# MIT-SPARK/Kimera-Semantics

Hardware: NVIDIA B200
Metric: depth_frames_per_s (higher is better)
Workload: dtype f32

## Files before the change

include/ksg.h:

```cpp
#ifndef KSG_H_
#define KSG_H_

#include <stddef.h>
#include <stdint.h>

#ifdef __cplusplus
extern "C" {
#endif

#define KSG_ABI_VERSION 1

enum {
  KSG_OK = 0,
  KSG_ERR_INVALID_ARGUMENT = 1,
  KSG_ERR_CUDA = 2,
  KSG_ERR_POOL_FULL = 3,
  KSG_ERR_SCRATCH_FULL = 4,
  KSG_ERR_INDEX_RANGE = 5,
  KSG_ERR_NO_DEVICE = 6
};

enum { KSG_INTEGRATOR_MERGED = 0, KSG_INTEGRATOR_FAST = 1 };
enum { KSG_COLOR_MODE_COLOR = 0, KSG_COLOR_MODE_SEMANTIC = 1, KSG_COLOR_MODE_SEMANTIC_PROBABILITY = 2 };
enum { KSG_ORDER_MIXED = 0, KSG_ORDER_SORTED = 1 };
// ... 143 lines not shown

int32_t ksg_reset(ksg_integrator* h);

int32_t ksg_owner_mask(int32_t voxels_per_side, int32_t shard_rank, int32_t shard_count, int64_t n,
                       const int32_t* block_index, uint8_t* mask);

int64_t ksg_unordered_map_schedule(int64_t n, int64_t* bucket_count_after_insert);

#define KSG_NUM_PHASES 7
int32_t ksg_set_profiling(ksg_integrator* h, int32_t enable);
int32_t ksg_get_profile(ksg_integrator* h, double* phase_ms , int64_t* frames,
                        int64_t* kernel_launches , int64_t* library_calls );

int64_t ksg_debug_tile_times(ksg_integrator* h, int32_t enable, int64_t capacity, int64_t* records_and_cycles);

int64_t ksg_debug_fast_timeline(ksg_integrator* h, int64_t* out80 , int64_t* sweeps, double* clock_khz);

int32_t ksg_debug_chain_sum(const float* terms, int64_t n, float s0, float* result);

const char* ksg_build_info(void);

#ifdef __cplusplus
}
#endif
#endif
```

kimera_semantics_b200/capi.py:

```python
from __future__ import annotations

import ctypes as C
import os
from typing import Dict, Optional

import numpy as np

KSG_ABI_VERSION = 1
KSG_INTEGRATOR_MERGED = 0
KSG_INTEGRATOR_FAST = 1
KSG_COLOR_MODE_COLOR = 0
KSG_COLOR_MODE_SEMANTIC = 1
KSG_COLOR_MODE_SEMANTIC_PROBABILITY = 2
KSG_ORDER_MIXED = 0
KSG_ORDER_SORTED = 1
KSG_BUNDLE_ORDER_CANONICAL = 0
KSG_BUNDLE_ORDER_LIBSTDCXX = 1

KSG_STATUS = {0: "OK", 1: "INVALID_ARGUMENT", 2: "CUDA", 3: "POOL_FULL", 4: "SCRATCH_FULL", 5: "INDEX_RANGE",
              6: "NO_DEVICE"}


class KsgConfig(C.Structure):
    _fields_ = [
# ... 413 lines not shown

    def set_profiling(self, enable: bool):
        self._check(self.lib.ksg_set_profiling(self.handle, int(enable)), "ksg_set_profiling")

    def get_profile(self) -> Dict[str, float]:
        ms = (C.c_double * 7)()
        frames, launches, libcalls = C.c_int64(), C.c_int64(), C.c_int64()
        self._check(self.lib.ksg_get_profile(self.handle, ms, C.byref(frames), C.byref(launches), C.byref(libcalls)), "ksg_get_profile")
        out = {n: float(ms[i]) for i, n in enumerate(self.PHASES)}
        out["frames"] = int(frames.value)
        out["kernel_launches"] = int(launches.value)
        out["library_calls"] = int(libcalls.value)
        return out

    def fast_timeline(self) -> Dict[str, object]:
        out = (C.c_int64 * 80)()
        sweeps, khz = C.c_int64(), C.c_double()
        n = int(self.lib.ksg_debug_fast_timeline(self.handle, out, C.byref(sweeps), C.byref(khz)))
        if n == 0:
            return {}
        t = [int(v) for v in out]
        us = lambda a, b: (t[b] - t[a]) / (khz.value / 1e3)
        ns = int(sweeps.value)
        return {"sweeps": ns, "compact_us": us(0, 1), "ray_setup_us": us(1, 2),
                "sweep_us": [us(2 + i, 3 + i) for i in range(max(0, min(ns, 48)))],
                "commit_emit_us": us(52, 53), "tile_count_us": us(53, 54), "tile_alloc_block_init_us": us(54, 55), "scatter_us": us(55, 56),
                "solve_kernel_us": us(0, 56),
                "phase0_us": {"file_shared_slot_visitors": us(0, 57) if t[57] else None, "sort_shared_slots": us(57, 58) if t[58] else None,
                              "scan_cast_counts": us(58 if t[58] else 0, 59), "compaction": us(59, 1)},
                "debug": {"max_ray_setup_us": t[64] / (khz.value / 1e3), "max_ray_setup_insert_us": t[65] / (khz.value / 1e3),
                          "max_ray_eval_us": t[67] / (khz.value / 1e3), "ray_evals": t[68], "blocks_evaluated": t[69], "blocks_materialised": t[70],
                          "ray_evals_that_changed": t[71], "max_shared_slot_visitors": t[72], "shared_slot_visitors": t[73],
                          "shared_slots": t[74], "rays": t[75],
                          "max_setup_after_loads_us": t[76] / (khz.value / 1e3), "max_setup_after_init_us": t[77] / (khz.value / 1e3),
                          "max_setup_after_loop_us": t[78] / (khz.value / 1e3), "max_eval_first_block_loads_us": t[79] / (khz.value / 1e3)}}

    def sync(self):
        self._check(self.lib.ksg_sync(self.handle), "ksg_sync")

    def reset(self):
        self._check(self.lib.ksg_reset(self.handle), "ksg_reset")

    def num_blocks(self) -> int:
        return int(self.lib.ksg_num_blocks(self.handle))

    def export(self) -> Dict[str, np.ndarray]:
        return export_arrays(self.lib, self.handle, "ksg", self.cfg.voxels_per_side, self.cfg.num_labels)

    def import_blocks(self, exp: Dict[str, np.ndarray]):
        a = {k: np.ascontiguousarray(v) for k, v in exp.items()}
# ... 78 lines not shown
```

kimera_semantics_b200/csrc/ksg_api.cu:

```cuda
#include <cuda_runtime.h>
#include <cub/cub.cuh>

#include <algorithm>
#include <cmath>
#include <cstdio>
#include <cstring>
#include <string>
#include <unordered_map>
#include <utility>
#include <vector>

#include "../../include/ksg.h"
#include "ksg_kernels.cuh"
#include "ksg_chain.cuh"
#include "ksg_hot.cuh"
#include "ksg_bundle_order.cuh"
#include "ksg_fast.cuh"
#include "ksg_fast3.cuh"
#include "ksg_voxel.cuh"
#include "ksg_merge.cuh"
#include "ksg_eval.cuh"
#include "ksg_mesh.cuh"

using namespace ksg;
// ... 99 lines not shown
  size_t cub_temp_bytes = 0;

  uint8_t* h_stage = nullptr;
  size_t h_stage_bytes = 0;
  uint8_t* d_in = nullptr;
  size_t d_in_bytes = 0;

  uint8_t* d_exp = nullptr;
  size_t d_exp_bytes = 0;
  int* d_exp_slots = nullptr;
  int exp_slots_cap = 0;

  bool fast_v2 = false;
  FastCounters* d_fc = nullptr;
  FastCounters* h_fc = nullptr;
  int *blk_cnt = nullptr, *blk_off = nullptr, *warp_cnt = nullptr, *warp_off = nullptr, *seq_of_i = nullptr;
  uint32_t* keys32 = nullptr;
  int *tile_cnt = nullptr, *tile_slot = nullptr;
  TileDesc* tile_list = nullptr;
  int solve_grid = 0, apply_fast_smem = 0;
  int solver = 3;
  int solve_threads = kSolveThreads;
  int group0 = kGroup0, group_mul = 4;
  Cand* cand16 = nullptr;
  OvfEnt* ovf = nullptr;
  RayRec* rayrec = nullptr;
  int ovf_cap = 0;
  int *mixed_list = nullptr, *m_list = nullptr, *blk_run = nullptr;
  VoxelUpdate *d_log_head = nullptr, *h_log_head = nullptr;
  float *d_log_prior = nullptr, *h_log_prior = nullptr;
// ... 79 lines not shown
  return KSG_OK;
}

template <typename Tp>
cudaError_t dmalloc(Tp** p, size_t count) { return cudaMalloc((void**)p, std::max<size_t>(count, 1) * sizeof(Tp)); }

void free_all(ksg_integrator* h) {
  cudaSetDevice(h->device);
  void* ptrs[] = {h->map.ht_keys, h->map.ht_slot, h->map.new_list, h->map.pool, h->map.slot_key, h->map.touched_stamp,
                  h->map.touched_list, h->d_luts, h->d_cnt, h->pt_pC, h->pt_pG, h->pt_label, h->pt_flags, h->pt_color, h->pt_key,
                  h->flags8, h->is_last, h->pix_list, h->point_of_seq, h->sq_keys, h->sq_keys_out, h->iota,
                  h->start_next, h->start_min, h->clear_ff, h->clear_00, h->start_table, h->cast_seq, h->ray_param, h->ray_label, h->ray_flags,
                  h->ray_color, h->nsteps, h->H, h->L, h->ray_state, h->ext_off, h->eval_sweep, h->ob.slot_stamp, h->ob.cand_pos, h->ob.bkt, h->ob.cand_val, h->ob.cand_order,
                  h->ob.cand_next, h->ob.table, h->ks_sorted, h->seq_sorted, h->bstart, h->bundle_f, h->hist,
                  h->tmp, h->tmp4, h->b_key, h->b_base, h->bord_hash, h->bord_scratch, h->d_scan_tot, h->bundle_f2, h->d_hot_segs, h->d_hot_counts, h->d_hot_chunk_seg, h->d_hot_guess, h->d_hot_sums,
                  h->d_hot_tables, h->d_hot_prior, h->d_hot_same, h->tile_debug, h->d_gridbar, h->d_fc, h->blk_cnt, h->blk_off, h->warp_cnt, h->warp_off, h->seq_of_i, h->keys32,
                  h->tile_cnt, h->tile_slot, h->tile_list, h->cand16, h->ovf, h->rayrec, h->mixed_list, h->m_list, h->blk_run, h->stamp64, h->d_log_head, h->d_log_prior, h->vq.long_items, h->vq.counters, h->rec_a, h->rec_b, h->tile_begin, h->cub_temp, h->d_in, h->d_exp, h->d_exp_slots};
  for (void* p : ptrs) if (p) cudaFree(p);
  if (h->h_cnt_base) cudaFreeHost(h->h_cnt_base);
  if (h->h_log_head) cudaFreeHost(h->h_log_head);
  if (h->h_log_prior) cudaFreeHost(h->h_log_prior);
  if (h->h_fc_base) cudaFreeHost(h->h_fc_base);
  for (int i = 0; i < 2; ++i) {
    if (h->ev_frame_s[i]) cudaEventDestroy(h->ev_frame_s[i]);
    if (h->ev_copy[i]) cudaEventDestroy(h->ev_copy[i]);
    if (h->ev_free[i]) cudaEventDestroy(h->ev_free[i]);
    if (h->d_in2[i]) cudaFree(h->d_in2[i]);
    if (h->h_stage2[i]) cudaFreeHost(h->h_stage2[i]);
  }
  if (h->copy_stream) cudaStreamDestroy(h->copy_stream);
  if (h->ev_fork) cudaEventDestroy(h->ev_fork);
// ... 203 lines not shown
      h->set_offset = 0;
      KSG_CUDA(cudaMemsetAsync(h->start_table, 0xFF, sizeof(uint32_t) * kSetSize, s));
      KSG_CUDA(cudaMemsetAsync(h->ob.table, 0xFF, sizeof(uint32_t) * kSetSize, s));
    }
  }
  FastFrame f{};
  f.cfg = h->dc; f.T = T; f.in = fin; f.in.pix_list = nullptr; f.in.point_of_seq = nullptr;
  f.luts = h->d_luts; f.cnt = h->d_cnt; f.fc = h->d_fc; f.map = h->map; f.ob = h->ob;
  f.sb = StartBuf{h->start_head, h->start_next, h->start_min, h->start_max, h->start_val, h->start_mixed, h->start_table};
  f.set_offset = h->set_offset;
  f.capacity = cap;
  f.n_count_blocks = (cap + kCountBlock - 1) / kCountBlock;
  f.vec_ok = in.d_depth ? (((uintptr_t)in.d_depth % 16 == 0 && (uintptr_t)in.d_label_img % 4 == 0) ? 1 : 0) : 0;
  f.frame_stamp = h->frame_stamp;
  f.profile = h->profiling ? 1 : 0;
  f.seq_of_i = sorted ? h->seq_of_i : nullptr;
  f.block_cnt = h->blk_cnt; f.block_off = h->blk_off; f.warp_cnt = h->warp_cnt; f.warp_off = h->warp_off;
  f.pt_pG = h->pt_pG; f.pt_label = h->pt_label; f.pt_flags = h->pt_flags; f.pt_color = h->pt_color; f.pt_key = h->pt_key;
  f.cast_flag = h->flags8;
  f.cast_seq = h->cast_seq; f.ray_param = h->ray_param; f.ray_label = h->ray_label; f.ray_flags = h->ray_flags; f.ray_color = h->ray_color;
  f.nsteps = h->nsteps; f.H = h->H; f.L = h->L; f.ray_state = h->ray_state; f.ext_off = h->ext_off; f.eval_sweep = h->eval_sweep;
  f.rec = h->rec_a; f.rec_cap = h->rec_cap; f.keys = h->keys32;
  f.tile_cnt = h->tile_cnt; f.tile_slot = h->tile_slot; f.tile_list = h->tile_list; f.tile_cap = h->tile_cap;
  f.o3.cand = h->cand16; f.o3.ext_base = h->ob.ext_base; f.o3.cand_cap = h->ob.cand_cap; f.o3.slot_cnt = h->ob.slot_cnt; f.o3.bkt = h->ob.bkt;
  f.o3.head = h->ob.head; f.o3.ovf = h->ovf; f.o3.ovf_cap = h->ovf_cap; f.o3.stamp_max = h->stamp64; f.o3.stamp_min = h->stamp64 + kSetSize; f.o3.table = h->ob.table;
  f.rayrec = h->rayrec; f.blk_run = h->blk_run;
  f.log_head = h->d_log_head; f.log_prior = h->d_log_prior; f.log_cap = h->log_cap;
  f.group0 = h->group0; f.group_mul = h->group_mul;
  f.s_base = h->start_head; f.s_hmin = h->start_val; f.s_hmax = (uint32_t*)(h->clear_00 + (size_t)kSetSize * 5);
  f.s_visits = (int*)(h->clear_00 + (size_t)kSetSize * 9); f.mixed_list = h->mixed_list; f.m_list = h->m_list;
  const bool s3 = h->solver == 3;

  if (h->profiling) {
    cudaEventRecord(h->ev[0], s);
    KSG_CUDA(cudaMemsetAsync(h->d_fc->dbg, 0, sizeof(h->d_fc->dbg), s));
  }
  KSG_CUDA(cudaMemsetAsync(h->clear_ff, 0xFF, (size_t)kSetSize * 16, s));
  KSG_CUDA(cudaMemsetAsync(h->clear_00, 0x00, (size_t)kSetSize * (s3 ? 13 : 5), s));
  KSG_CUDA(cudaMemsetAsync(h->start_min, 0x7F, sizeof(int) * kSetSize, s));
  const int B = 256;
  ++h->n_launches;
  if (in.d_depth) k_fast_count<<<f.n_count_blocks, 256, 0, s>>>(f);
  else k_fast_reset<<<1, 1, 0, s>>>(f);
  if (sorted) {
    h->n_launches += 3;
    if (in.d_depth) k_fast_sqnorm<<<f.n_count_blocks, 256, 0, s>>>(f, h->sq_keys);
    else k_fast_sqnorm_points<<<grid_for(cap, B), B, 0, s>>>(f, h->sq_keys);
    k_fast_pad_keys<<<grid_for(cap, B), B, 0, s>>>(h->d_cnt, cap, h->sq_keys);
    size_t tb = h->cub_temp_bytes;
    ++h->n_libcalls;
// ... 1583 lines not shown
    const uint64_t key = pack_key(bi);
    for (int z = 0; z < vps; ++z)
      for (int y = 0; y < vps; ++y)
        for (int x = 0; x < vps; ++x) {
          const int tile = (x / T) + tps * ((y / T) + tps * (z / T));
          mask[b * V + (size_t)x + (size_t)vps * ((size_t)y + (size_t)vps * z)] = tile_owner(key, tile, count) == shard_rank ? 1 : 0;
        }
  }
  return KSG_OK;
}

int32_t ksg_set_profiling(ksg_integrator* h, int32_t enable) {
  if (!h) return KSG_ERR_INVALID_ARGUMENT;
  cudaSetDevice(h->device);
  if (enable && !h->ev[0]) for (auto& e : h->ev) cudaEventCreate(&e);
  h->profiling = enable != 0;
  for (double& m : h->phase_ms) m = 0.0;
  h->prof_frames = 0; h->n_launches = 0; h->n_libcalls = 0;
  return KSG_OK;
}
int32_t ksg_get_profile(ksg_integrator* h, double* phase_ms, int64_t* frames, int64_t* kernel_launches, int64_t* library_calls) {
  if (!h) return KSG_ERR_INVALID_ARGUMENT;
  if (phase_ms) for (int p = 0; p < KSG_NUM_PHASES; ++p) phase_ms[p] = h->phase_ms[p];
  if (frames) *frames = h->prof_frames;
  if (kernel_launches) *kernel_launches = h->n_launches;
  if (library_calls) *library_calls = h->n_libcalls;
  return KSG_OK;
}

namespace {
// ... 28 lines not shown
    if (cudaMalloc((void**)&h->tile_debug, sizeof(long long) * 2 * (size_t)h->tile_cap) != cudaSuccess) { h->tile_debug = nullptr; return 0; }
  }
  const int64_t n = std::min<int64_t>(h->h_cnt->n_tiles, h->tile_cap);
  if (h->tile_debug && records_and_cycles && capacity >= n && n > 0)
    cudaMemcpy(records_and_cycles, h->tile_debug, sizeof(long long) * 2 * n, cudaMemcpyDeviceToHost);
  if (!enable && h->tile_debug) { cudaFree(h->tile_debug); h->tile_debug = nullptr; }
  return n;
}

int64_t ksg_debug_fast_timeline(ksg_integrator* h, int64_t* out64, int64_t* sweeps, double* clock_khz) {
  if (!h || !out64 || !h->h_fc) return 0;
  cudaSetDevice(h->device);
  if (h->n_pend > 0) finish_frame(h, nullptr);
  for (int i = 0; i < kTimelineSlots; ++i) out64[i] = (int64_t)h->h_fc->timeline[i];
  for (int i = 0; i < 16; ++i) out64[kTimelineSlots + i] = (int64_t)h->h_fc->dbg[i];
  if (sweeps) *sweeps = h->h_fc->sweeps_last;
  if (clock_khz) *clock_khz = h->clock_khz;
  return kTimelineSlots + 16;
}

int32_t ksg_clear_map(ksg_integrator* h) {
  if (!h) return KSG_ERR_INVALID_ARGUMENT;
  auto fail = [&](int c, const char* m) { return h->fail(c, m); };
  KSG_CUDA(cudaSetDevice(h->device));
  KSG_CUDA(cudaDeviceSynchronize());
  { const int rcp = finish_frame(h, nullptr); if (rcp) return rcp; }
  cudaStream_t s = h->own_stream;
  KSG_CUDA(cudaMemsetAsync(h->map.ht_keys, 0xFF, sizeof(uint64_t) * h->ht_cap, s));
  KSG_CUDA(cudaMemsetAsync(h->map.ht_slot, 0xFF, sizeof(int) * h->ht_cap, s));
  KSG_CUDA(cudaMemsetAsync(h->map.touched_stamp, 0, sizeof(int) * h->ht_cap, s));
  if (h->tile_cnt) KSG_CUDA(cudaMemsetAsync(h->tile_cnt, 0, sizeof(int) * (size_t)h->ht_cap * h->dc.tiles_per_block, s));
  KSG_CUDA(cudaMemsetAsync(&h->d_cnt->pool_count, 0, sizeof(int), s));
  KSG_CUDA(cudaMemsetAsync(&h->d_cnt->n_blocks_touched, 0, sizeof(int), s));
// ... 17 lines not shown
```

kimera_semantics_b200/csrc/ksg_fast.cuh:

```cuda
#pragma once
#include "ksg_kernels.cuh"

namespace ksg {

static constexpr int kCountBlock = 1024;
static constexpr int kEvalBlock = 512;
static constexpr int kSolveThreads = 1024;
static constexpr int kFastKeyCap = 4096;
static constexpr int kFastPref = 1024;
static constexpr int kTimelineSlots = 64;

struct FastCounters {
  unsigned int ticket_count, ticket_eval;
  unsigned int gridbar;
  int sweep_base;
  int sweeps_last;
  int tile_cursor;
  int n_tile_list;
  int pool_base;
  unsigned long long rec_cursor;
  int ovf_count;
  int n_mixed;
  int m_cursor;
  int log_count;
  long long timeline[kTimelineSlots];
// ... 25 lines not shown
  DevCfg cfg;
  Xform T;
  FrameIn in;
  const Luts* luts;
  Counters* cnt;
  FastCounters* fc;
  MapRef map;
  ObsBuf ob;
  StartBuf sb;
  uint64_t set_offset;
  int capacity;
  int n_count_blocks;
  int vec_ok;
  int frame_stamp;
  int profile;
  const int* seq_of_i;
  int* block_cnt; int* block_off;
  int* warp_cnt; int* warp_off;
  float4* pt_pG; uint8_t* pt_label; uint8_t* pt_flags; uint32_t* pt_color; uint64_t* pt_key; uint8_t* cast_flag;
  int* cast_seq; float4* ray_param; uint8_t* ray_label; uint8_t* ray_flags; uint32_t* ray_color;
  int* nsteps; int* H; int* L; RayState* ray_state; long long* ext_off; int* eval_sweep;
  uint64_t* rec; long long rec_cap;
  uint32_t* keys;
  int* tile_cnt;
  int* tile_slot;
  TileDesc* tile_list; long long tile_cap;
  Obs3 o3;
  RayRec* rayrec;
  int* blk_run;
  int group0, group_mul;
// ... 282 lines not shown
          f.mixed_list[atomicAdd(&f.fc->n_mixed, 1)] = (int)slot;
        }
      }
    }
  }
  if (seq < f.capacity) f.cast_flag[seq] = cast;
  const unsigned m = __ballot_sync(0xffffffffu, cast != 0);
  if (lane == 0) __stcg(&f.warp_cnt[seq >> 5], __popc(m));
  if (blockIdx.x == 0 && threadIdx.x == 0) f.fc->gridbar = 0;
}

__device__ __forceinline__ void warp_sort_i32(int* a, int n, int lane) {
  int n2 = 1;
  while (n2 < n) n2 <<= 1;
  const int half = n2 >> 1;
  for (int k = 2; k <= n2; k <<= 1) {
    const int hk = k >> 1;
    for (int t = lane; t < half; t += 32) {
      const int blk = t / hk, o = t - blk * hk;
      const int i = blk * k + o, p = blk * k + (k - 1 - o);
      if (p < n) { const int x = a[i], y = a[p]; if (x > y) { a[i] = y; a[p] = x; } }
    }
    __syncwarp();
    for (int j = k >> 2; j > 0; j >>= 1) {
      for (int t = lane; t < half; t += 32) {
        const int i = (t / j) * 2 * j + (t % j), p = i + j;
        if (p < n) { const int x = a[i], y = a[p]; if (x > y) { a[i] = y; a[p] = x; } }
      }
      __syncwarp();
    }
  }
}

__device__ __forceinline__ void solve_barrier(unsigned int* bar, unsigned int& epoch) {
  __syncthreads();
  if (threadIdx.x == 0) {
    __threadfence();
    const unsigned int target = (++epoch) * gridDim.x;
    atomicAdd(bar, 1u);
    while (((volatile unsigned int*)bar)[0] < target) {}
    __threadfence();
  }
  __syncthreads();
}
__device__ __forceinline__ void dbg_max(const FastFrame& f, int k, long long v) { if (f.profile) atomicMax((unsigned long long*)&f.fc->dbg[k], (unsigned long long)v); }
__device__ __forceinline__ void dbg_add(const FastFrame& f, int k, long long v) { if (f.profile) atomicAdd((unsigned long long*)&f.fc->dbg[k], (unsigned long long)v); }
__device__ __forceinline__ void timeline_mark(const FastFrame& f, int slot) {
  if (f.profile && blockIdx.x == 0 && threadIdx.x == 0 && slot < kTimelineSlots) f.fc->timeline[slot] = clock64();
}

__device__ __forceinline__ void fast_ray_setup(const FastFrame& f, int r, int n_cast) {
  const DevCfg& cfg = f.cfg;
  int h = 0;
  if (r < n_cast) {
    const int seq = f.cast_seq[r];
    const float4 p = f.pt_pG[seq];
    const uint8_t fl = f.pt_flags[seq];
    f.ray_param[r] = p;
    f.ray_label[r] = f.pt_label[seq];
    f.ray_flags[r] = fl;
    f.ray_color[r] = f.pt_color[seq];
// ... 487 lines not shown
```

kimera_semantics_b200/csrc/ksg_fast3.cuh:

```cuda
#pragma once
#include "ksg_fast.cuh"

namespace ksg {

struct __align__(16) Cand { uint64_t vkey; int pos; int tog; };
struct __align__(16) OvfEnt { uint64_t order_perf; uint32_t hi; int next; };
struct __align__(16) RayRec { int H, L, nsteps, eval_sweep; };
static constexpr int kBkt3 = 32;
static constexpr int kOvfPending = -2;
static constexpr int kSortPerWarp = 1024;

__device__ __forceinline__ Cand ld_cand(const Cand* p) {
  const int4 v = __ldcg((const int4*)p);
  Cand c; c.vkey = ((uint64_t)(uint32_t)v.y << 32) | (uint32_t)v.x; c.pos = v.z; c.tog = v.w;
  return c;
}
__device__ __forceinline__ void st_cand(Cand* p, uint64_t vkey, int pos, int tog) {
  __stcg((int4*)p, make_int4((int)(uint32_t)vkey, (int)(uint32_t)(vkey >> 32), pos, tog));
}
__device__ __forceinline__ void st_cand_state(Cand* p, int pos, int tog) { __stcg((int2*)p + 1, make_int2(pos, tog)); }
__device__ __forceinline__ uint64_t cand_value(uint64_t vkey, uint64_t offset) { return (uint64_t)index_hash(unpack_key(vkey)) + offset; }
__device__ __forceinline__ uint64_t make_entry(bool on, uint64_t order, uint64_t v) { return (on ? kEntPerf : 0ull) | (order << 13) | (v >> kSetBits); }
__device__ __forceinline__ long long cand_index3(const Obs3& o, const long long* ext_off, int r, int s) {
  if (s < kH0) return (long long)r * kH0 + s;
// ... 3 lines not shown

static constexpr uint32_t kSweepCap = 0x7FFFFFFFu;
__device__ __forceinline__ void stamp_toggle(const Obs3& o, uint32_t slot, int sweep, int r) {
  atomicMax((unsigned long long*)&o.stamp_max[slot], ((unsigned long long)(uint32_t)sweep << 32) | (uint32_t)r);
  atomicMin((unsigned long long*)&o.stamp_min[slot], ((unsigned long long)(kSweepCap - (uint32_t)sweep) << 32) | (uint32_t)r);
}
__device__ __forceinline__ bool stamp_dirty(const Obs3& o, uint32_t slot, int last, int r) {
  const unsigned long long a = __ldcg((const unsigned long long*)&o.stamp_max[slot]);
  const unsigned long long b = __ldcg((const unsigned long long*)&o.stamp_min[slot]);
  const int sk = (int)(a >> 32);
  if (sk > last) return true;
  if (sk < last) return false;
  return !((uint32_t)(b >> 32) == kSweepCap - (uint32_t)sk && (uint32_t)a == (uint32_t)r && (uint32_t)b == (uint32_t)r);
}

__device__ __forceinline__ int cand_insert_raw(int* slot_cnt, uint64_t* bkt, int* head, OvfEnt* ovf, int ovf_cap, int* ovf_count, Counters* cnt,
                                            uint32_t slot, uint64_t entry) {
  const int idx = atomicAdd(&slot_cnt[slot], 1);
  if (idx < kBkt3) { const int pos = (int)slot * kBkt3 + idx; __stcg(&bkt[pos], entry); return pos; }
  const int id = atomicAdd(ovf_count, 1);
  if (id >= ovf_cap) { set_err(cnt, 4); return -2; }
  OvfEnt* e = &ovf[id];
  __stcg(&e->next, kOvfPending);
  __stcg(&e->order_perf, (entry & kEntPerf) | ((entry >> 13) & ((1ull << kEntOrderBits) - 1)));
  __stcg(&e->hi, (uint32_t)(entry & 0x1FFFull));
  const int old = atomicExch(&head[slot], id);
  __stcg(&e->next, old);
  return -3 - id;
}
__device__ __forceinline__ int cand_insert3(const FastFrame& f, uint32_t slot, uint64_t entry) {
  return cand_insert_raw(f.o3.slot_cnt, f.o3.bkt, f.o3.head, f.o3.ovf, f.o3.ovf_cap, &f.fc->ovf_count, f.cnt, slot, entry);
}

__device__ __forceinline__ int latest_performed_before_raw(const uint64_t* bkt, const int* slot_cnt, const int* head, const OvfEnt* ovf, int ovf_cap,
                                                        uint32_t slot, uint64_t my_order) {
  const ulonglong2* b = (const ulonglong2*)(bkt + (size_t)slot * kBkt3);
  const int total = __ldcg(&slot_cnt[slot]);
  ulonglong2 v[4];
#pragma unroll
  for (int q = 0; q < 4; ++q) v[q] = __ldcg(b + q);
  const int n = total < kBkt3 ? total : kBkt3;
  long long best = -1;
  int best_hi = -1;
#pragma unroll
  for (int q = 0; q < 4; ++q) scan_entries(v[q], 2 * q, n, my_order, best, best_hi);
#pragma unroll 1
// ... 7 lines not shown
    int guard = total - kBkt3 + 8;
#pragma unroll 1
    for (int id = __ldcg(&head[slot]); id >= 0 && id < ovf_cap && guard-- > 0; id = __ldcg(&ovf[id].next)) {
      const uint64_t op = __ldcg(&ovf[id].order_perf);
      const uint64_t eo = op & ~kEntPerf;
      if ((op & kEntPerf) && eo < my_order && (long long)eo > best) { best = (long long)eo; best_hi = (int)__ldcg(&ovf[id].hi); }
    }
  }
  return best_hi;
}
__device__ __forceinline__ int latest_performed_before3(const Obs3& o, uint32_t slot, uint64_t my_order) {
  return latest_performed_before_raw(o.bkt, o.slot_cnt, o.head, o.ovf, o.ovf_cap, slot, my_order);
}
__device__ __forceinline__ bool later_performed_exists_raw(const uint64_t* bkt, const int* slot_cnt, const int* head, const OvfEnt* ovf, int ovf_cap,
                                                        uint32_t slot, uint64_t my_order) {
  const int total = __ldcg(&slot_cnt[slot]);
  const int n = total < kBkt3 ? total : kBkt3;
  const uint64_t* b = bkt + (size_t)slot * kBkt3;
  bool later = false;
#pragma unroll 1
  for (int j = 0; j < n; ++j) {
    const uint64_t e = __ldcg(&b[j]);
    if ((e & kEntPerf) && ((e >> 13) & ((1ull << kEntOrderBits) - 1)) > my_order) later = true;
  }
  if (total > kBkt3) {
    int guard = total - kBkt3 + 8;
#pragma unroll 1
    for (int id = __ldcg(&head[slot]); id >= 0 && id < ovf_cap && !later && guard-- > 0; id = __ldcg(&ovf[id].next)) {
      const uint64_t op = __ldcg(&ovf[id].order_perf);
      if ((op & kEntPerf) && (op & ~kEntPerf) > my_order) later = true;
    }
  }
  return later;
}
__device__ __forceinline__ bool later_performed_exists3(const Obs3& o, uint32_t slot, uint64_t my_order) {
  return later_performed_exists_raw(o.bkt, o.slot_cnt, o.head, o.ovf, o.ovf_cap, slot, my_order);
}

// ... 121 lines not shown
  for (int r = r_lo + (threadIdx.x >> 5) * gridDim.x + blockIdx.x; r < r_hi; r += warps_total) {
    const int4 rr = __ldcg((const int4*)&f.rayrec[r]);
    int h = rr.x;
    const int old = rr.y, n = rr.z, last = rr.w;
    int fd = 0x7fffffff;
    if (last == 0) fd = 0;
    else {
      const int upto = (old < h - 1) ? old : h - 1;
      for (int s = lane; s <= upto; s += 32) {
        const Cand c = ld_cand(&o.cand[cand_index3(o, f.ext_off, r, s)]);
        const uint32_t slot = (uint32_t)cand_value(c.vkey, f.set_offset) & kSetMask;
        if (stamp_dirty(o, slot, last, r)) { fd = s; break; }
      }
      for (int d = 16; d > 0; d >>= 1) { const int t = __shfl_xor_sync(0xffffffffu, fd, d); fd = t < fd ? t : fd; }
    }
    if (fd == 0x7fffffff) continue;
    const long long t_eval = f.profile ? clock64() : 0;
    int n_blocks_eval = 0, n_blocks_mat = 0;
    int s0, blen;
    block_of_step(fd, s0, blen);
    long long base_ci = cand_index3(o, f.ext_off, r, s0);
    int run = (s0 == 0) ? 0 : __ldcg(&f.blk_run[base_ci >> 4]);
    int U = -1;
    while (s0 < n && U < 0) {
      const int cend = (s0 + blen < n) ? s0 + blen : n;
      ++n_blocks_eval;
      if (s0 >= h) {
        ++n_blocks_mat;
        int ok = 1;
        if (lane == 0 && s0 >= kH0 && (s0 & (s0 - 1)) == 0) {
          const int k = 31 - __clz(s0 >> 4);
// ... 39 lines not shown
      bool coll[2];
#pragma unroll
      for (int q = 0; q < 2; ++q) {
        const int s = s0 + q * 32 + lane;
        c[q].vkey = 0; c[q].pos = -2; c[q].tog = 0; v[q] = 0; coll[q] = false;
        if (s < cend) { c[q] = ld_cand(&o.cand[base_ci + q * 32 + lane]); v[q] = cand_value(c[q].vkey, f.set_offset); }
      }
#pragma unroll
      for (int q = 0; q < 2; ++q) {
        const int s = s0 + q * 32 + lane;
        if (s < cend) {
          const uint32_t slot = (uint32_t)v[q] & kSetMask;
          const uint32_t stale = o.table[slot];
          const int hi = latest_performed_before3(o, slot, ((uint64_t)r << kOrderStepBits) | (uint64_t)s);
          coll[q] = (hi >= 0) ? ((uint32_t)hi == (uint32_t)(v[q] >> kSetBits)) : (stale == (uint32_t)(v[q] >> kSetBits));
        }
      }
      const unsigned bits0 = __ballot_sync(0xffffffffu, coll[0]), bits1 = __ballot_sync(0xffffffffu, coll[1]);
      if (f.profile && lane == 0 && n_blocks_eval == 1) dbg_max(f, 15, clock64() - t_eval);
      int brk = -1;
      for (int jj = 0; s0 + jj < cend; ++jj) {
        const unsigned bit = (jj < 32) ? ((bits0 >> jj) & 1u) : ((bits1 >> (jj - 32)) & 1u);
        if (bit) ++run; else run = 0;
        if (run > cfg.maxc) { brk = s0 + jj; break; }
      }
      const int perf_end = (brk >= 0) ? brk : cend;
#pragma unroll
      for (int q = 0; q < 2; ++q) {
        const int s = s0 + q * 32 + lane;
        if (s < perf_end && s >= old)
// ... 4 lines not shown
      s0 = cend;
      if (s0 < n) { int nb; block_of_step(s0, s0, nb); blen = nb; if (s0 < h) base_ci = cand_index3(o, f.ext_off, r, s0); }
    }
    if (U < 0) U = n;
    if (U < old) {
      for (int s = U + lane; s < old; s += 32) {
        const long long ci = cand_index3(o, f.ext_off, r, s);
        Cand c = ld_cand(&o.cand[ci]);
        const uint64_t v = cand_value(c.vkey, f.set_offset);
        set_performed3(f, c, ci, (uint32_t)v & kSetMask, ((uint64_t)r << kOrderStepBits) | (uint64_t)s, v, false, sweep, r);
      }
    }
    if (lane == 0) {
      if (U != old) { f.rayrec[r].L = U; cnt->changed[sweep & 3] = 1; }
      f.rayrec[r].eval_sweep = sweep;
      if (f.profile) { dbg_max(f, 3, clock64() - t_eval); dbg_add(f, 4, 1); dbg_add(f, 5, n_blocks_eval); dbg_add(f, 6, n_blocks_mat); if (U != old) dbg_add(f, 7, 1); }
    }
  }
}

template <int PASS>
__device__ __forceinline__ void fast3_walk_performed(const FastFrame& f, int n_cast, int n_tiles) {
  constexpr int G = 8;
  const Obs3& o = f.o3;
  const DevCfg& cfg = f.cfg;
  const int groups_total = (gridDim.x * blockDim.x) / G;
  const int gl = threadIdx.x % G;
  const int gt = ((((threadIdx.x >> 5) * gridDim.x + blockIdx.x) << 5) | (threadIdx.x & 31));
  for (int r = gt / G; r < n_cast; r += groups_total) {
    const int U = __ldcg(&f.rayrec[r].L);
    for (int s = gl; s < U; s += G) {
// ... 21 lines not shown
        if (idx >= 0 && idx < n_tiles && at >= 0) f.keys[__ldcg(&f.tile_list[idx].off) + at] = (uint32_t)rec;
      }
    }
  }
}

__global__ void __launch_bounds__(kSolveThreads, 1) k_fast_solve3(FastFrame f, int max_sweeps) {
  unsigned int epoch = 0;
  unsigned int* bar = &f.fc->gridbar;
  const int lane = threadIdx.x & 31;
  const int gtid = (((threadIdx.x >> 5) * gridDim.x + blockIdx.x) << 5) | lane;
  const int gthreads = gridDim.x * blockDim.x;
  Counters* cnt = f.cnt;
  const int n_points = cnt->n_points;
  int tl = 0;
  timeline_mark(f, tl++);
  extern __shared__ int s_sort[];
  const int n_mixed = ((volatile int*)&f.fc->n_mixed)[0];
  if (n_mixed > 0) {
    for (int seq = gtid; seq < n_points; seq += gthreads) {
      const uint64_t v = f.pt_key[seq];
      if (v == ~0ull) continue;
      const uint32_t slot = (uint32_t)v & kSetMask;
      if (f.s_hmin[slot] != f.s_hmax[slot]) f.m_list[f.s_base[slot] + f.sb.next[seq]] = seq;
    }
    solve_barrier(bar, epoch);
    timeline_mark(f, 57);
    const int warps_total = gthreads >> 5;
    int* scratch = s_sort + (threadIdx.x >> 5) * kSortPerWarp;
    for (int mi = (threadIdx.x >> 5) * gridDim.x + blockIdx.x; mi < n_mixed; mi += warps_total) {
      const int slot = f.mixed_list[mi];
      const int n = __ldcg(&f.s_visits[slot]);
      int* seg = f.m_list + __ldcg(&f.s_base[slot]);
      int* a = seg;
      if (n <= kSortPerWarp) { for (int i = lane; i < n; i += 32) scratch[i] = __ldcg(&seg[i]); a = scratch; }
      __syncwarp();
      warp_sort_i32(a, n, lane);
      for (int i = 1 + lane; i < n; i += 32) {
        const int pa = a[i - 1], pb = a[i];
        if (f.pt_key[pa] != f.pt_key[pb]) { f.cast_flag[pb] = 1; atomicAdd(&f.warp_cnt[pb >> 5], 1); }
      }
      __syncwarp();
      if (f.profile && lane == 0) { dbg_max(f, 8, n); dbg_add(f, 9, n); }
    }
    solve_barrier(bar, epoch);
    timeline_mark(f, 58);
  }
  if (blockIdx.x == 0) {
    const int n_warps32 = (f.capacity + 31) >> 5;
    const int total = block_scan_array(f.warp_cnt, f.warp_off, n_warps32);
    if (threadIdx.x == 0) cnt->n_cast = total;
  }
  solve_barrier(bar, epoch);
  timeline_mark(f, 59);
  const int n_cast = ((volatile int*)&cnt->n_cast)[0];
  for (int base = (gtid & ~31); base < n_points; base += gthreads) {
    const int seq = base + lane;
    const bool c = seq < n_points && __ldcg(&f.cast_flag[seq]) != 0;
    const unsigned m = __ballot_sync(0xffffffffu, c);
    if (c) f.cast_seq[__ldcg(&f.warp_off[seq >> 5]) + __popc(m & ((1u << lane) - 1u))] = seq;
  }
  const int sweep_base0 = ((volatile int*)&f.fc->sweep_base)[0];
  const bool wrap = false;
  solve_barrier(bar, epoch);
  timeline_mark(f, tl++);
  for (int r0 = (gtid & ~31); r0 < n_cast; r0 += gthreads) fast3_ray_setup(f, r0 + lane, n_cast);
  solve_barrier(bar, epoch);
  timeline_mark(f, tl++);
  int sweep = (wrap ? 0 : sweep_base0);
  sweep = (sweep + 4) & ~3;
  const int first_sweep = sweep + 1;
  bool failed = false;
  int g_lo = 0, g_size = f.group0 > 0 ? f.group0 : kGroup0;
  while (g_lo < n_cast && !failed) {
    const int g_hi = (g_lo + g_size < n_cast) ? g_lo + g_size : n_cast;
    bool converged = false;
    for (int it = 0; it < max_sweeps; ++it) {
      ++sweep;
      fast3_sweep(f, sweep, g_lo, g_hi, (WarpDdaScratch*)(s_sort + (threadIdx.x >> 5) * kSortPerWarp));
      solve_barrier(bar, epoch);
      if (tl < kTimelineSlots - 12) timeline_mark(f, tl++);
      const int changed = ((volatile int*)cnt->changed)[sweep & 3];
      const int err = ((volatile int*)&cnt->err)[0];
      if (err) { failed = true; break; }
      if (!changed) { converged = true; break; }
    }
    if (!converged) failed = true;
    g_lo = g_hi;
    g_size = (g_size < (1 << 28)) ? g_size * (f.group_mul > 1 ? f.group_mul : 4) : g_size;
  }
  if (gtid == 0) {
    cnt->last_sweep = sweep;
    f.fc->sweep_base = sweep;
    f.fc->sweeps_last = sweep - first_sweep + 1;
    if (failed && !((volatile int*)&cnt->err)[0]) set_err(cnt, 2 );
    if (f.profile) f.fc->timeline[kTimelineSlots - 1] = tl;
  }
  tl = kTimelineSlots - 12;
  timeline_mark(f, tl++);
  if (!failed) fast3_walk_performed<1>(f, n_cast, 0);
  solve_barrier(bar, epoch);
  timeline_mark(f, tl++);
  timeline_mark(f, tl++);
  const bool ok = ((volatile int*)&cnt->err)[0] == 0 && !failed;
  const int n_new_all = ((volatile int*)&cnt->n_new_blocks)[0];
  const int n_new = n_new_all < f.map.new_cap ? n_new_all : f.map.new_cap;
  const int pool_base = ((volatile int*)&cnt->pool_count)[0];
  const int n_tiles = (int)min((long long)((volatile int*)&f.fc->n_tile_list)[0], f.tile_cap);
  for (int base = (gtid & ~31); base < n_tiles; base += gthreads) {
    const int idx = base + lane;
    int n = 0;
    uint32_t tk = 0;
    if (idx < n_tiles) { tk = f.tile_list[idx].tk; n = __ldcg(&f.tile_cnt[tk]); }
    const long long off = (long long)warp_alloc(&f.fc->rec_cursor, (unsigned long long)n);
    if (idx < n_tiles) {
      const int pos = (int)(tk / (uint32_t)f.cfg.tiles_per_block);
      const int old = atomicExch(&f.map.touched_stamp[pos], f.frame_stamp);
      if (old != f.frame_stamp) f.map.touched_list[atomicAdd(&cnt->n_blocks_touched, 1)] = pos;
      const bool owned = f.cfg.shard_count <= 1 ||
                         tile_owner(f.map.ht_keys[pos], (int)(tk % (uint32_t)f.cfg.tiles_per_block), f.cfg.shard_count) == f.cfg.shard_rank;
      if (off + n > f.rec_cap) { set_err(cnt, 4); n = 0; }
      f.tile_list[idx].n = owned ? n : -n;
      f.tile_list[idx].off = off;
    }
  }
  if (ok) fast_block_init(f, n_new, pool_base);
  solve_barrier(bar, epoch);
  timeline_mark(f, tl++);
  const bool ok2 = ((volatile int*)&cnt->err)[0] == 0 && !failed;
  if (!failed) fast3_walk_performed<2>(f, n_cast, ok2 ? n_tiles : 0);
  if (gtid == 0) {
    int add = n_new;
    if (pool_base + add > f.map.max_blocks) add = f.map.max_blocks - pool_base;
    if (ok) cnt->pool_count = pool_base + (add > 0 ? add : 0);
    cnt->n_tiles = ok2 ? n_tiles : 0;
    cnt->n_records = ((volatile unsigned long long*)&f.fc->rec_cursor)[0];
    f.fc->tile_cursor = 0;
    f.fc->n_tile_list = 0;
    f.fc->rec_cursor = 0;
    f.fc->ovf_count = 0;
    if (f.profile) { f.fc->dbg[10] = n_mixed; f.fc->dbg[11] = n_cast; }
    f.fc->n_mixed = 0;
    f.fc->m_cursor = 0;
    f.fc->log_count = 0;
  }
  timeline_mark(f, tl++);
}

}
```

Measured before the change: 2175.

## Add shared-memory profiling counters and vectorize slot scans and sort indexing

Profiling counters now accumulate in shared memory and are flushed once per block before each grid barrier. New per-sweep and overflow statistics are exposed through an extended timeline buffer. Separately, the bitonic warp sort replaces divisions with shifts, later_performed_exists_raw reads bucket entries as 128-bit vector loads in groups of four, and the cast-flag key comparison loop is unrolled four ways. The non-profiling changes target integer divide cost and load latency in hot loops, at the price of the bucket scan always loading eight entries even when fewer are valid.

```diff
diff --git a/include/ksg.h b/include/ksg.h
--- a/include/ksg.h
+++ b/include/ksg.h
@@ -181,7 +181,7 @@
 
 int64_t ksg_debug_tile_times(ksg_integrator* h, int32_t enable, int64_t capacity, int64_t* records_and_cycles);
 
-int64_t ksg_debug_fast_timeline(ksg_integrator* h, int64_t* out80 , int64_t* sweeps, double* clock_khz);
+int64_t ksg_debug_fast_timeline(ksg_integrator* h, int64_t* out112 , int64_t* sweeps, double* clock_khz);
 
 int32_t ksg_debug_chain_sum(const float* terms, int64_t n, float s0, float* result);
 
diff --git a/kimera_semantics_b200/capi.py b/kimera_semantics_b200/capi.py
--- a/kimera_semantics_b200/capi.py
+++ b/kimera_semantics_b200/capi.py
@@ -451,7 +451,7 @@
         return out
 
     def fast_timeline(self) -> Dict[str, object]:
-        out = (C.c_int64 * 80)()
+        out = (C.c_int64 * 112)()
         sweeps, khz = C.c_int64(), C.c_double()
         n = int(self.lib.ksg_debug_fast_timeline(self.handle, out, C.byref(sweeps), C.byref(khz)))
         if n == 0:
@@ -470,7 +470,10 @@
                           "ray_evals_that_changed": t[71], "max_shared_slot_visitors": t[72], "shared_slot_visitors": t[73],
                           "shared_slots": t[74], "rays": t[75],
                           "max_setup_after_loads_us": t[76] / (khz.value / 1e3), "max_setup_after_init_us": t[77] / (khz.value / 1e3),
-                          "max_setup_after_loop_us": t[78] / (khz.value / 1e3), "max_eval_first_block_loads_us": t[79] / (khz.value / 1e3)}}
+                          "max_setup_after_loop_us": t[78] / (khz.value / 1e3), "max_eval_first_block_loads_us": t[79] / (khz.value / 1e3),
+                          "overflow_entries": t[80], "max_slot_count": t[81], "max_overflow_chain_walked": t[82],
+                          "sweep_clean_rays": [t[84 + 2 * i] for i in range(max(0, min(ns, 14)))],
+                          "sweep_ray_evals": [t[85 + 2 * i] for i in range(max(0, min(ns, 14)))]}}
 
     def sync(self):
         self._check(self.lib.ksg_sync(self.handle), "ksg_sync")
diff --git a/kimera_semantics_b200/csrc/ksg_api.cu b/kimera_semantics_b200/csrc/ksg_api.cu
--- a/kimera_semantics_b200/csrc/ksg_api.cu
+++ b/kimera_semantics_b200/csrc/ksg_api.cu
@@ -137,6 +137,7 @@
   bool fast_v2 = false;
   FastCounters* d_fc = nullptr;
   FastCounters* h_fc = nullptr;
+  long long* d_prof = nullptr;
   int *blk_cnt = nullptr, *blk_off = nullptr, *warp_cnt = nullptr, *warp_off = nullptr, *seq_of_i = nullptr;
   uint32_t* keys32 = nullptr;
   int *tile_cnt = nullptr, *tile_slot = nullptr;
@@ -246,7 +247,7 @@
                   h->ray_color, h->nsteps, h->H, h->L, h->ray_state, h->ext_off, h->eval_sweep, h->ob.slot_stamp, h->ob.cand_pos, h->ob.bkt, h->ob.cand_val, h->ob.cand_order,
                   h->ob.cand_next, h->ob.table, h->ks_sorted, h->seq_sorted, h->bstart, h->bundle_f, h->hist,
                   h->tmp, h->tmp4, h->b_key, h->b_base, h->bord_hash, h->bord_scratch, h->d_scan_tot, h->bundle_f2, h->d_hot_segs, h->d_hot_counts, h->d_hot_chunk_seg, h->d_hot_guess, h->d_hot_sums,
-                  h->d_hot_tables, h->d_hot_prior, h->d_hot_same, h->tile_debug, h->d_gridbar, h->d_fc, h->blk_cnt, h->blk_off, h->warp_cnt, h->warp_off, h->seq_of_i, h->keys32,
+                  h->d_hot_tables, h->d_hot_prior, h->d_hot_same, h->tile_debug, h->d_gridbar, h->d_fc, h->d_prof, h->blk_cnt, h->blk_off, h->warp_cnt, h->warp_off, h->seq_of_i, h->keys32,
                   h->tile_cnt, h->tile_slot, h->tile_list, h->cand16, h->ovf, h->rayrec, h->mixed_list, h->m_list, h->blk_run, h->stamp64, h->d_log_head, h->d_log_prior, h->vq.long_items, h->vq.counters, h->rec_a, h->rec_b, h->tile_begin, h->cub_temp, h->d_in, h->d_exp, h->d_exp_slots};
   for (void* p : ptrs) if (p) cudaFree(p);
   if (h->h_cnt_base) cudaFreeHost(h->h_cnt_base);
@@ -480,6 +481,7 @@
   f.vec_ok = in.d_depth ? (((uintptr_t)in.d_depth % 16 == 0 && (uintptr_t)in.d_label_img % 4 == 0) ? 1 : 0) : 0;
   f.frame_stamp = h->frame_stamp;
   f.profile = h->profiling ? 1 : 0;
+  f.prof = h->d_prof;
   f.seq_of_i = sorted ? h->seq_of_i : nullptr;
   f.block_cnt = h->blk_cnt; f.block_off = h->blk_off; f.warp_cnt = h->warp_cnt; f.warp_off = h->warp_off;
   f.pt_pG = h->pt_pG; f.pt_label = h->pt_label; f.pt_flags = h->pt_flags; f.pt_color = h->pt_color; f.pt_key = h->pt_key;
@@ -500,6 +502,7 @@
   if (h->profiling) {
     cudaEventRecord(h->ev[0], s);
     KSG_CUDA(cudaMemsetAsync(h->d_fc->dbg, 0, sizeof(h->d_fc->dbg), s));
+    KSG_CUDA(cudaMemsetAsync(h->d_prof, 0, sizeof(long long) * kProfSlots, s));
   }
   KSG_CUDA(cudaMemsetAsync(h->clear_ff, 0xFF, (size_t)kSetSize * 16, s));
   KSG_CUDA(cudaMemsetAsync(h->clear_00, 0x00, (size_t)kSetSize * (s3 ? 13 : 5), s));
@@ -2113,6 +2116,10 @@
   if (!h) return KSG_ERR_INVALID_ARGUMENT;
   cudaSetDevice(h->device);
   if (enable && !h->ev[0]) for (auto& e : h->ev) cudaEventCreate(&e);
+  if (enable && h->d_fc && !h->d_prof) {
+    if (cudaMalloc(&h->d_prof, sizeof(long long) * kProfSlots) != cudaSuccess) { h->d_prof = nullptr; return KSG_ERR_CUDA; }
+    cudaMemset(h->d_prof, 0, sizeof(long long) * kProfSlots);
+  }
   h->profiling = enable != 0;
   for (double& m : h->phase_ms) m = 0.0;
   h->prof_frames = 0; h->n_launches = 0; h->n_libcalls = 0;
@@ -2171,9 +2178,12 @@
   if (h->n_pend > 0) finish_frame(h, nullptr);
   for (int i = 0; i < kTimelineSlots; ++i) out64[i] = (int64_t)h->h_fc->timeline[i];
   for (int i = 0; i < 16; ++i) out64[kTimelineSlots + i] = (int64_t)h->h_fc->dbg[i];
+  long long prof[kProfSlots] = {};
+  if (h->d_prof) cudaMemcpy(prof, h->d_prof, sizeof(prof), cudaMemcpyDeviceToHost);
+  for (int i = 0; i < kProfSlots; ++i) out64[kTimelineSlots + 16 + i] = (int64_t)prof[i];
   if (sweeps) *sweeps = h->h_fc->sweeps_last;
   if (clock_khz) *clock_khz = h->clock_khz;
-  return kTimelineSlots + 16;
+  return kTimelineSlots + 16 + kProfSlots;
 }
 
 int32_t ksg_clear_map(ksg_integrator* h) {
diff --git a/kimera_semantics_b200/csrc/ksg_fast.cuh b/kimera_semantics_b200/csrc/ksg_fast.cuh
--- a/kimera_semantics_b200/csrc/ksg_fast.cuh
+++ b/kimera_semantics_b200/csrc/ksg_fast.cuh
@@ -9,6 +9,8 @@
 static constexpr int kFastKeyCap = 4096;
 static constexpr int kFastPref = 1024;
 static constexpr int kTimelineSlots = 64;
+static constexpr int kProfSlots = 32;
+static constexpr int kProfSweeps = (kProfSlots - 4) / 2;
 
 struct FastCounters {
   unsigned int ticket_count, ticket_eval;
@@ -64,6 +66,7 @@
   int vec_ok;
   int frame_stamp;
   int profile;
+  long long* prof;
   const int* seq_of_i;
   int* block_cnt; int* block_off;
   int* warp_cnt; int* warp_off;
@@ -376,17 +379,18 @@
   int n2 = 1;
   while (n2 < n) n2 <<= 1;
   const int half = n2 >> 1;
-  for (int k = 2; k <= n2; k <<= 1) {
-    const int hk = k >> 1;
+  for (int lk = 1; (1 << lk) <= n2; ++lk) {
+    const int k = 1 << lk, lhk = lk - 1;
     for (int t = lane; t < half; t += 32) {
-      const int blk = t / hk, o = t - blk * hk;
+      const int blk = t >> lhk, o = t & ((1 << lhk) - 1);
       const int i = blk * k + o, p = blk * k + (k - 1 - o);
       if (p < n) { const int x = a[i], y = a[p]; if (x > y) { a[i] = y; a[p] = x; } }
     }
     __syncwarp();
-    for (int j = k >> 2; j > 0; j >>= 1) {
+    for (int lj = lk - 2; lj >= 0; --lj) {
+      const int j = 1 << lj;
       for (int t = lane; t < half; t += 32) {
-        const int i = (t / j) * 2 * j + (t % j), p = i + j;
+        const int i = ((t >> lj) << (lj + 1)) + (t & (j - 1)), p = i + j;
         if (p < n) { const int x = a[i], y = a[p]; if (x > y) { a[i] = y; a[p] = x; } }
       }
       __syncwarp();
@@ -405,8 +409,31 @@
   }
   __syncthreads();
 }
-__device__ __forceinline__ void dbg_max(const FastFrame& f, int k, long long v) { if (f.profile) atomicMax((unsigned long long*)&f.fc->dbg[k], (unsigned long long)v); }
-__device__ __forceinline__ void dbg_add(const FastFrame& f, int k, long long v) { if (f.profile) atomicAdd((unsigned long long*)&f.fc->dbg[k], (unsigned long long)v); }
+static constexpr int kDbgShared = 20;
+static constexpr unsigned kDbgAddMask = (1u << 4) | (1u << 5) | (1u << 6) | (1u << 7) | (1u << 9);
+__shared__ unsigned long long s_dbg[kDbgShared];
+__device__ __forceinline__ void dbg_max(const FastFrame& f, int k, long long v) { if (f.profile) atomicMax(&s_dbg[k], (unsigned long long)v); }
+__device__ __forceinline__ void dbg_add(const FastFrame& f, int k, long long v) { if (f.profile) atomicAdd(&s_dbg[k], (unsigned long long)v); }
+__device__ __forceinline__ void prof_init(const FastFrame& f) {
+  if (!f.profile) return;
+  if (threadIdx.x < kDbgShared) s_dbg[threadIdx.x] = 0;
+  __syncthreads();
+}
+__device__ __forceinline__ void prof_flush(const FastFrame& f, int sweep_idx) {
+  if (!f.profile) return;
+  __syncthreads();
+  const int k = threadIdx.x;
+  if (k < kDbgShared) {
+    const unsigned long long v = s_dbg[k];
+    if (v) {
+      if (k < 16) {
+        if ((kDbgAddMask >> k) & 1u) atomicAdd((unsigned long long*)&f.fc->dbg[k], v); else atomicMax((unsigned long long*)&f.fc->dbg[k], v);
+      } else if (k < 18) atomicMax((unsigned long long*)&f.prof[k - 15], v);
+      else if (sweep_idx >= 0 && sweep_idx < kProfSweeps) atomicAdd((unsigned long long*)&f.prof[4 + 2 * sweep_idx + (k - 18)], v);
+      s_dbg[k] = 0;
+    }
+  }
+}
 __device__ __forceinline__ void timeline_mark(const FastFrame& f, int slot) {
   if (f.profile && blockIdx.x == 0 && threadIdx.x == 0 && slot < kTimelineSlots) f.fc->timeline[slot] = clock64();
 }
diff --git a/kimera_semantics_b200/csrc/ksg_fast3.cuh b/kimera_semantics_b200/csrc/ksg_fast3.cuh
--- a/kimera_semantics_b200/csrc/ksg_fast3.cuh
+++ b/kimera_semantics_b200/csrc/ksg_fast3.cuh
@@ -41,22 +41,20 @@
   return !((uint32_t)(b >> 32) == kSweepCap - (uint32_t)sk && (uint32_t)a == (uint32_t)r && (uint32_t)b == (uint32_t)r);
 }
 
-__device__ __forceinline__ int cand_insert_raw(int* slot_cnt, uint64_t* bkt, int* head, OvfEnt* ovf, int ovf_cap, int* ovf_count, Counters* cnt,
-                                            uint32_t slot, uint64_t entry) {
-  const int idx = atomicAdd(&slot_cnt[slot], 1);
-  if (idx < kBkt3) { const int pos = (int)slot * kBkt3 + idx; __stcg(&bkt[pos], entry); return pos; }
-  const int id = atomicAdd(ovf_count, 1);
-  if (id >= ovf_cap) { set_err(cnt, 4); return -2; }
-  OvfEnt* e = &ovf[id];
+__device__ __forceinline__ int cand_insert3(const FastFrame& f, uint32_t slot, uint64_t entry) {
+  const Obs3& o = f.o3;
+  const int idx = atomicAdd(&o.slot_cnt[slot], 1);
+  if (f.profile) dbg_max(f, 16, idx + 1);
+  if (idx < kBkt3) { const int pos = (int)slot * kBkt3 + idx; __stcg(&o.bkt[pos], entry); return pos; }
+  const int id = atomicAdd(&f.fc->ovf_count, 1);
+  if (id >= o.ovf_cap) { set_err(f.cnt, 4); return -2; }
+  OvfEnt* e = &o.ovf[id];
   __stcg(&e->next, kOvfPending);
   __stcg(&e->order_perf, (entry & kEntPerf) | ((entry >> 13) & ((1ull << kEntOrderBits) - 1)));
   __stcg(&e->hi, (uint32_t)(entry & 0x1FFFull));
-  const int old = atomicExch(&head[slot], id);
+  const int old = atomicExch(&o.head[slot], id);
   __stcg(&e->next, old);
   return -3 - id;
-}
-__device__ __forceinline__ int cand_insert3(const FastFrame& f, uint32_t slot, uint64_t entry) {
-  return cand_insert_raw(f.o3.slot_cnt, f.o3.bkt, f.o3.head, f.o3.ovf, f.o3.ovf_cap, &f.fc->ovf_count, f.cnt, slot, entry);
 }
 
 __device__ __forceinline__ int latest_performed_before_raw(const uint64_t* bkt, const int* slot_cnt, const int* head, const OvfEnt* ovf, int ovf_cap,
@@ -94,14 +92,26 @@
 }
 __device__ __forceinline__ bool later_performed_exists_raw(const uint64_t* bkt, const int* slot_cnt, const int* head, const OvfEnt* ovf, int ovf_cap,
                                                         uint32_t slot, uint64_t my_order) {
+  const ulonglong2* b = (const ulonglong2*)(bkt + (size_t)slot * kBkt3);
   const int total = __ldcg(&slot_cnt[slot]);
+  ulonglong2 v[4];
+#pragma unroll
+  for (int q = 0; q < 4; ++q) v[q] = __ldcg(b + q);
   const int n = total < kBkt3 ? total : kBkt3;
-  const uint64_t* b = bkt + (size_t)slot * kBkt3;
   bool later = false;
 #pragma unroll 1
-  for (int j = 0; j < n; ++j) {
-    const uint64_t e = __ldcg(&b[j]);
-    if ((e & kEntPerf) && ((e >> 13) & ((1ull << kEntOrderBits) - 1)) > my_order) later = true;
+  for (int q0 = 0;;) {
+#pragma unroll
+    for (int q = 0; q < 4; ++q) {
+      const uint64_t e2[2] = {v[q].x, v[q].y};
+#pragma unroll
+      for (int k = 0; k < 2; ++k)
+        if (2 * (q0 + q) + k < n && (e2[k] & kEntPerf) && ((e2[k] >> 13) & ((1ull << kEntOrderBits) - 1)) > my_order) later = true;
+    }
+    q0 += 4;
+    if (2 * q0 >= n) break;
+#pragma unroll
+    for (int q = 0; q < 4; ++q) v[q] = __ldcg(b + q0 + q);
   }
   if (total > kBkt3) {
     int guard = total - kBkt3 + 8;
@@ -253,7 +263,7 @@
       }
       for (int d = 16; d > 0; d >>= 1) { const int t = __shfl_xor_sync(0xffffffffu, fd, d); fd = t < fd ? t : fd; }
     }
-    if (fd == 0x7fffffff) continue;
+    if (fd == 0x7fffffff) { if (f.profile && lane == 0) dbg_add(f, 18, 1); continue; }
     const long long t_eval = f.profile ? clock64() : 0;
     int n_blocks_eval = 0, n_blocks_mat = 0;
     int s0, blen;
@@ -323,6 +333,7 @@
           const uint32_t stale = o.table[slot];
           const int hi = latest_performed_before3(o, slot, ((uint64_t)r << kOrderStepBits) | (uint64_t)s);
           coll[q] = (hi >= 0) ? ((uint32_t)hi == (uint32_t)(v[q] >> kSetBits)) : (stale == (uint32_t)(v[q] >> kSetBits));
+          if (f.profile) { const int tot = __ldcg(&o.slot_cnt[slot]); if (tot > kBkt3) dbg_max(f, 17, tot - kBkt3); }
         }
       }
       const unsigned bits0 = __ballot_sync(0xffffffffu, coll[0]), bits1 = __ballot_sync(0xffffffffu, coll[1]);
@@ -357,7 +368,7 @@
     if (lane == 0) {
       if (U != old) { f.rayrec[r].L = U; cnt->changed[sweep & 3] = 1; }
       f.rayrec[r].eval_sweep = sweep;
-      if (f.profile) { dbg_max(f, 3, clock64() - t_eval); dbg_add(f, 4, 1); dbg_add(f, 5, n_blocks_eval); dbg_add(f, 6, n_blocks_mat); if (U != old) dbg_add(f, 7, 1); }
+      if (f.profile) { dbg_max(f, 3, clock64() - t_eval); dbg_add(f, 4, 1); dbg_add(f, 5, n_blocks_eval); dbg_add(f, 6, n_blocks_mat); if (U != old) dbg_add(f, 7, 1); dbg_add(f, 19, 1); }
     }
   }
 }
@@ -409,6 +420,7 @@
   Counters* cnt = f.cnt;
   const int n_points = cnt->n_points;
   int tl = 0;
+  prof_init(f);
   timeline_mark(f, tl++);
   extern __shared__ int s_sort[];
   const int n_mixed = ((volatile int*)&f.fc->n_mixed)[0];
@@ -419,6 +431,7 @@
       const uint32_t slot = (uint32_t)v & kSetMask;
       if (f.s_hmin[slot] != f.s_hmax[slot]) f.m_list[f.s_base[slot] + f.sb.next[seq]] = seq;
     }
+    prof_flush(f, -1);
     solve_barrier(bar, epoch);
     timeline_mark(f, 57);
     const int warps_total = gthreads >> 5;
@@ -428,16 +441,30 @@
       const int n = __ldcg(&f.s_visits[slot]);
       int* seg = f.m_list + __ldcg(&f.s_base[slot]);
       int* a = seg;
-      if (n <= kSortPerWarp) { for (int i = lane; i < n; i += 32) scratch[i] = __ldcg(&seg[i]); a = scratch; }
+      if (n <= kSortPerWarp) {
+#pragma unroll 4
+        for (int i = lane; i < n; i += 32) scratch[i] = __ldcg(&seg[i]);
+        a = scratch;
+      }
       __syncwarp();
       warp_sort_i32(a, n, lane);
-      for (int i = 1 + lane; i < n; i += 32) {
-        const int pa = a[i - 1], pb = a[i];
-        if (f.pt_key[pa] != f.pt_key[pb]) { f.cast_flag[pb] = 1; atomicAdd(&f.warp_cnt[pb >> 5], 1); }
+      for (int i0 = 1 + lane; i0 < n; i0 += 4 * 32) {
+        int pb[4];
+        uint64_t ka[4], kb[4];
+#pragma unroll
+        for (int u = 0; u < 4; ++u) {
+          const int i = i0 + 32 * u;
+          pb[u] = -1; ka[u] = kb[u] = 0;
+          if (i < n) { pb[u] = a[i]; ka[u] = f.pt_key[a[i - 1]]; kb[u] = f.pt_key[pb[u]]; }
+        }
+#pragma unroll
+        for (int u = 0; u < 4; ++u)
+          if (pb[u] >= 0 && ka[u] != kb[u]) { f.cast_flag[pb[u]] = 1; atomicAdd(&f.warp_cnt[pb[u] >> 5], 1); }
       }
       __syncwarp();
       if (f.profile && lane == 0) { dbg_max(f, 8, n); dbg_add(f, 9, n); }
     }
+    prof_flush(f, -1);
     solve_barrier(bar, epoch);
     timeline_mark(f, 58);
   }
@@ -446,6 +473,7 @@
     const int total = block_scan_array(f.warp_cnt, f.warp_off, n_warps32);
     if (threadIdx.x == 0) cnt->n_cast = total;
   }
+  prof_flush(f, -1);
   solve_barrier(bar, epoch);
   timeline_mark(f, 59);
   const int n_cast = ((volatile int*)&cnt->n_cast)[0];
@@ -457,9 +485,11 @@
   }
   const int sweep_base0 = ((volatile int*)&f.fc->sweep_base)[0];
   const bool wrap = false;
+  prof_flush(f, -1);
   solve_barrier(bar, epoch);
   timeline_mark(f, tl++);
   for (int r0 = (gtid & ~31); r0 < n_cast; r0 += gthreads) fast3_ray_setup(f, r0 + lane, n_cast);
+  prof_flush(f, -1);
   solve_barrier(bar, epoch);
   timeline_mark(f, tl++);
   int sweep = (wrap ? 0 : sweep_base0);
@@ -473,6 +503,7 @@
     for (int it = 0; it < max_sweeps; ++it) {
       ++sweep;
       fast3_sweep(f, sweep, g_lo, g_hi, (WarpDdaScratch*)(s_sort + (threadIdx.x >> 5) * kSortPerWarp));
+      prof_flush(f, sweep - first_sweep);
       solve_barrier(bar, epoch);
       if (tl < kTimelineSlots - 12) timeline_mark(f, tl++);
       const int changed = ((volatile int*)cnt->changed)[sweep & 3];
@@ -494,6 +525,7 @@
   tl = kTimelineSlots - 12;
   timeline_mark(f, tl++);
   if (!failed) fast3_walk_performed<1>(f, n_cast, 0);
+  prof_flush(f, -1);
   solve_barrier(bar, epoch);
   timeline_mark(f, tl++);
   timeline_mark(f, tl++);
@@ -520,6 +552,7 @@
     }
   }
   if (ok) fast_block_init(f, n_new, pool_base);
+  prof_flush(f, -1);
   solve_barrier(bar, epoch);
   timeline_mark(f, tl++);
   const bool ok2 = ((volatile int*)&cnt->err)[0] == 0 && !failed;
@@ -533,6 +566,7 @@
     f.fc->tile_cursor = 0;
     f.fc->n_tile_list = 0;
     f.fc->rec_cursor = 0;
+    if (f.profile) f.prof[0] = f.fc->ovf_count;
     f.fc->ovf_count = 0;
     if (f.profile) { f.fc->dbg[10] = n_mixed; f.fc->dbg[11] = n_cast; }
     f.fc->n_mixed = 0;
```

Result: faster. 2532, median of 6 (+16.4%).
